# jumerckx/Monodepth2.jl

Measured on AMD Instinct MI355X. Metric: train-step images/sec, ResNet-18 416×128; 1/2/4/8 MI355X + roofline %, higher is better.
Workload: dtype fp32; 1 GPU; train_step resnet18 depth+pose decoders, 4-scale photometric loss, ADAM; batch_per_gpu=12, global_batch=12, height=128, width=416, parallelism=dp1

## Files before the change

include/md2.h:

```cpp
#ifndef MD2_H
#define MD2_H

#include <stddef.h>

#ifdef __cplusplus
extern "C" {
#endif

#define MD2_ABI_VERSION 2

#define MD2_OK 0
#define MD2_EINVAL 1
#define MD2_EHIP 2
#define MD2_ENOTSUP 3
#define MD2_ENOMEM 4
#define MD2_ESTATE 5

int md2_abi_version(void);
const char* md2_build_id(void);
const char* md2_last_error(void);
int md2_device_count(int* count);
int md2_memcpy_d2d(void* dst, const void* src, size_t bytes, void* stream);

#define MD2_MAX_SCALES 5
// ... 54 lines not shown
                        void* stream);
int md2_project_fwd(const float* points, int n, int w, int h, const float* K, const float* R,
                    const float* t, float* out, void* stream);
size_t md2_project_workspace_size(int n, int w, int h);
int md2_project_bwd(const float* points, int n, int w, int h, const float* K, const float* R,
                    const float* t, const float* dout, float* d_points, float* d_R, float* d_t,
                    void* workspace, void* stream);
int md2_grid_sample_border_fwd(const float* x, const float* grid, int n, int c, int hi, int wi,
                               int ho, int wo, float* out, void* stream);
int md2_grid_sample_border_bwd(const float* x, const float* grid, const float* dout, int n, int c,
                               int hi, int wi, int ho, int wo, float* d_grid, float* d_x,
                               void* stream);
size_t md2_smooth_loss_workspace_size(int n, int w, int h);
int md2_smooth_loss_fwd(const float* disp, const float* img, int n, int c, int h, int w,
                        float* loss, void* workspace, void* stream);
int md2_smooth_loss_bwd(const float* disp, const float* img, int n, int c, int h, int w,
                        float dloss, float* d_disp, void* workspace, void* stream);

typedef struct md2_warp_cfg {
  int n, c, width, height;
  int dw, dh;
  float K[9], invK[9];
  float min_depth, max_depth;
  long long x_sample_stride;
  long long x_frame_stride;
  int target, src0, src1;
} md2_warp_cfg;
size_t md2_warp_photometric_workspace_size(const md2_warp_cfg* cfg);
int md2_warp_photometric_fwd(const md2_warp_cfg* cfg, const float* disp, const float* Rt,
                             const float* x, const float* automask, float* loss_map,
                             signed char* sel_map, void* workspace, void* stream);
int md2_warp_photometric_bwd(const md2_warp_cfg* cfg, const float* disp, const float* Rt,
                             const float* x, const float* automask, const float* d_loss,
                             float* d_disp, float* d_Rt, void* workspace, void* stream);

int md2_png_info(const char* path, int* width, int* height, int* channels);
int md2_load_triplets_u8(const char* const* paths, int n, int width, int height,
                         const unsigned char* flip, unsigned char* out, int threads);
int md2_load_kitti_u8(const char* const* paths, int n, int height, int width,
                      const unsigned char* flip, unsigned char* out, int threads);

int md2_unorm8_to_float(const unsigned char* in, float* out, long long n, void* stream);

typedef struct md2_conv_desc {
  int n, cin, h, w, cout, kh, kw, stride, pad, reflect;
  int act;
} md2_conv_desc;

size_t md2_conv2d_workspace_size(const md2_conv_desc* d);
int md2_conv2d_fwd(const md2_conv_desc* d, const float* x, const float* w, const float* bias,
                   float* y, void* workspace, void* stream);
int md2_conv2d_dgrad(const md2_conv_desc* d, const float* dy, const float* w, float* dx,
                     void* workspace, void* stream);
int md2_conv2d_wgrad(const md2_conv_desc* d, const float* x, const float* dy, float* dw,
                     float* db, void* workspace, void* stream);
int md2_act_backward(const float* out, const float* dout, float* dpre, long long n, int act,
                     void* stream);

int md2_maxpool3s2_fwd(const float* x, int n, int c, int h, int w, float* y, unsigned char* arg,
                       void* stream);
int md2_maxpool3s2_bwd(const float* dy, const unsigned char* arg, int n, int c, int h, int w,
                       float* dx, void* stream);
int md2_upsample2_fwd(const float* x, int n, int c, int h, int w, float* y, void* stream);
int md2_upsample2_bwd(const float* dy, int n, int c, int h, int w, float* dx, void* stream);

int md2_mpi_embed_features(const float* feat, long long sample_stride, int n, int c, int h, int w,
                           const float* bins, int num_bins, int L, float* out, void* stream);
int md2_concat_channels(const float* a, int ca, const float* b, int cb, int n, long long hw,
                        float* out, void* stream);

int md2_mine_src_xyz(const float* disparity, int n_planes, int batch, int h, int w,
                     const float* invK, float* xyz, void* stream);
int md2_mine_tgt_xyz(const float* xyz_src, const float* pose, int n_planes, int batch, int h, int w,
                     float* xyz_tgt, void* stream);
int md2_mine_sample(const float* src, int c, const float* depth, const float* pose, int n_planes,
                    int batch, int h, int w, const float* K, const float* invK, float* out,
                    float* valid, void* stream);
int md2_plane_volume_rendering(const float* rgb, const float* sigma, const float* xyz, int n_planes,
                               int batch, int h, int w, float* rgb_out, float* transparency_acc,
                               float* weights, void* stream);
int md2_render_tgt_rgb_depth(const float* rgb, const float* sigma, const float* disparity,
                             const float* xyz_tgt, const float* pose, const float* invK,
                             const float* K, int n_planes, int batch, int h, int w, float* rgb_out,
                             float* depth, float* mask, void* stream);

typedef struct md2_model_cfg {
  int arch;
  int in_channels;
  int batch;
  int width, height;
  int n_levels;
  int scale_levels[MD2_MAX_SCALES];
  float K[9], invK[9];
  float min_depth, max_depth, disparity_smoothness;
  float scales[MD2_MAX_SCALES];
  int automasking;
  int target, src0, src1;
  int embedding_levels;
  int num_bins;
} md2_model_cfg;

typedef struct md2_model md2_model;

int md2_arch_param_count(const md2_model_cfg* cfg, long long* n_entries, long long* n_elems);
int md2_arch_param_info(const md2_model_cfg* cfg, int idx, char* name, int name_len, int* ndim,
                        int* shape4, long long* offset);
// ... 85 lines not shown
```

monodepth2.jl_amd/csrc/api.cpp:

```cpp
#include "../../include/md2.h"

#include <cmath>
#include <cstdlib>
#include <cstring>
#include <string>

#include "conv.h"
#include "loss_tail.h"
#include "mine.h"
#include "model.h"
#include "nn.h"

#include <algorithm>

#include <dlfcn.h>
#include <execinfo.h>
#include <csignal>
#include <unistd.h>

namespace md2 {
static struct sigaction g_prev_segv, g_prev_abrt;
static void segv_trace(int sig, siginfo_t* info, void* uctx) {
  void* frames[64];
  const int n = backtrace(frames, 64);
// ... 170 lines not shown
                        float* d_pose, void* stream) {
  MD2_CHECK_ARG(pose && dRt && d_pose && n > 0, "so3 bwd args");
  return launch_so3_bwd(pose, 2 * n, n, invert_mask, dRt, d_pose, 0, (hipStream_t)stream);
}

static ConvShape to_shape(const md2_conv_desc* d) {
  ConvShape s{};
  s.N = d->n;
  s.Cin = d->cin;
  s.H = d->h;
  s.W = d->w;
  s.Cout = d->cout;
  s.KH = d->kh;
  s.KW = d->kw;
  s.stride = d->stride;
  s.pad = d->pad;
  s.reflect = d->reflect;
  s.Ho = (d->h + 2 * d->pad - d->kh) / d->stride + 1;
  s.Wo = (d->w + 2 * d->pad - d->kw) / d->stride + 1;
  return s;
}

static size_t align_up(size_t b) { return (b + 255) & ~size_t(255); }

size_t md2_conv2d_workspace_size(const md2_conv_desc* d) {
  if (!d) return 0;
  const ConvShape s = to_shape(d);
  size_t packed = std::max(conv_fwd_packed_elems(s), conv_dgrad_packed_elems(s)) * sizeof(float);
  size_t slab = std::max(conv_fwd_workspace(s), std::max(conv_dgrad_workspace(s), conv_wgrad_workspace(s)));
  return align_up(packed) + align_up(slab);
}

int md2_conv2d_fwd(const md2_conv_desc* d, const float* x, const float* w, const float* bias,
                   float* y, void* workspace, void* stream) {
  MD2_CHECK_ARG(d && x && w && y && workspace, "conv2d_fwd args");
  const ConvShape s = to_shape(d);
  hipStream_t st = (hipStream_t)stream;
  float* packed = (float*)workspace;
  const size_t pbytes = align_up(std::max(conv_fwd_packed_elems(s), conv_dgrad_packed_elems(s)) * sizeof(float));
  MD2_TRY(conv_pack_fwd(s, w, packed, st));
  TensorIn in;
  in.p0 = x;
  in.c0 = s.Cin;
  in.bs0 = (long)s.Cin * s.H * s.W;
  TensorOut out;
  out.p0 = y;
  out.bs0 = (long)s.Cout * s.Ho * s.Wo;
  out.bias = bias;
  out.act = d->act;
  ConvWorkspace ws{(char*)workspace + pbytes, md2_conv2d_workspace_size(d) - pbytes};
  return conv_fwd(s, in, packed, out, ws, st);
}

int md2_conv2d_dgrad(const md2_conv_desc* d, const float* dy, const float* w, float* dx,
                     void* workspace, void* stream) {
  MD2_CHECK_ARG(d && dy && w && dx && workspace, "conv2d_dgrad args");
  const ConvShape s = to_shape(d);
  hipStream_t st = (hipStream_t)stream;
  float* packed = (float*)workspace;
  const size_t pbytes = align_up(std::max(conv_fwd_packed_elems(s), conv_dgrad_packed_elems(s)) * sizeof(float));
  MD2_TRY(conv_pack_dgrad(s, w, packed, st));
  TensorOut out;
  out.p0 = dx;
  out.bs0 = (long)s.Cin * s.H * s.W;
  ConvWorkspace ws{(char*)workspace + pbytes, md2_conv2d_workspace_size(d) - pbytes};
  return conv_dgrad(s, dy, packed, out, ws, st);
}

int md2_conv2d_wgrad(const md2_conv_desc* d, const float* x, const float* dy, float* dw,
                     float* db, void* workspace, void* stream) {
  MD2_CHECK_ARG(d && x && dy && dw && workspace, "conv2d_wgrad args");
  const ConvShape s = to_shape(d);
  const size_t pbytes = align_up(std::max(conv_fwd_packed_elems(s), conv_dgrad_packed_elems(s)) * sizeof(float));
  TensorIn in;
  in.p0 = x;
  in.c0 = s.Cin;
  in.bs0 = (long)s.Cin * s.H * s.W;
  ConvWorkspace ws{(char*)workspace + pbytes, md2_conv2d_workspace_size(d) - pbytes};
  return conv_wgrad(s, in, dy, dw, db, 0, ws, (hipStream_t)stream);
}

int md2_act_backward(const float* out, const float* dout, float* dpre, long long n, int act,
                     void* stream) {
  MD2_CHECK_ARG(out && dout && dpre && n >= 0, "act_backward args");
  return act_backward(out, dout, dpre, (long)n, act, (hipStream_t)stream);
}

int md2_adam(float* p, const float* g, float* adam_m, float* adam_v, long long n, float lr,
             float beta1, float beta2, float eps, int step, float grad_scale, void* stream) {
  MD2_CHECK_ARG(p && g && adam_m && adam_v && n > 0 && step >= 1, "adam args");
  const double bc1 = 1.0 - std::pow((double)beta1, step), bc2 = 1.0 - std::pow((double)beta2, step);
  return adam_step(p, g, adam_m, adam_v, (long)n, lr, beta1, beta2, eps, (float)bc1, (float)bc2,
                   grad_scale, (hipStream_t)stream);
}

int md2_maxpool3s2_fwd(const float* x, int n, int c, int h, int w, float* y, unsigned char* arg,
                       void* stream) {
  MD2_CHECK_ARG(x && y && arg && n > 0 && c > 0 && h > 0 && w > 0, "maxpool3s2_fwd args");
  return maxpool_fwd(x, n, c, h, w, y, arg, (h + 1) / 2, (w + 1) / 2, (hipStream_t)stream);
}
int md2_maxpool3s2_bwd(const float* dy, const unsigned char* arg, int n, int c, int h, int w,
                       float* dx, void* stream) {
  MD2_CHECK_ARG(dy && arg && dx && n > 0 && c > 0 && h > 0 && w > 0, "maxpool3s2_bwd args");
  return maxpool_bwd(dy, arg, n, c, h, w, (h + 1) / 2, (w + 1) / 2, dx, (hipStream_t)stream);
}
int md2_upsample2_fwd(const float* x, int n, int c, int h, int w, float* y, void* stream) {
  MD2_CHECK_ARG(x && y && n > 0 && c > 0 && h > 0 && w > 0, "upsample2_fwd args");
  return upsample2_fwd(x, n, c, h, w, y, (hipStream_t)stream);
}
int md2_mpi_embed_features(const float* feat, long long sample_stride, int n, int c, int h, int w,
                           const float* bins, int num_bins, int L, float* out, void* stream) {
  MD2_CHECK_ARG(feat && bins && out && n > 0 && c > 0 && h > 0 && w > 0 && num_bins > 0 && L >= 0 &&
                    sample_stride >= (long long)c * h * w, "mpi_embed_features args");
  return mpi_embed_features(feat, (long)sample_stride, n, c, h, w, bins, num_bins, L, out,
                            (hipStream_t)stream);
}
int md2_concat_channels(const float* a, int ca, const float* b, int cb, int n, long long hw,
                        float* out, void* stream) {
  MD2_CHECK_ARG(a && b && out && ca > 0 && cb > 0 && n > 0 && hw > 0, "concat_channels args");
// ... 306 lines not shown
```

monodepth2.jl_amd/csrc/conv.hip:

```cpp
#include "conv_plan.h"
#include "conv_lds.h"

namespace md2 {

struct PackOne {
  const float* w;
  float* out;
  int mode, tap, layout, Cout, Cin, KK, Kpad, Mpad;
  int Cinw;
};

__device__ __forceinline__ long packed_index(int k, int m, int layout, int Mpad) {
  return layout ? ((long)(k >> 4) * Mpad + m) * 16 + (k & 15) : (long)k * Mpad + m;
}
__device__ __forceinline__ void pack_store(float* out, int k, int m, int layout, int Mpad, float v) {
  if (layout == 2) {
    uint16_t* o = reinterpret_cast<uint16_t*>(out);
    uint32_t h, md, l;
    split3(v, h, md, l);
    const long base = ((long)(k >> 4) * 3 * Mpad + m) * 16 + (k & 15), ps = (long)Mpad * 16;
    o[base] = (uint16_t)(h >> 16);
    o[base + ps] = (uint16_t)(md >> 16);
    o[base + 2 * ps] = (uint16_t)(l >> 16);
  } else {
// ... 200 lines not shown
  return p;
}

HaloPlan plan_halo(const ConvShape& s, int mode) {
  HaloPlan h;
  static const int on = tuning_knob("MD2_HALO", 1);
  static const int target = tuning_knob("MD2_HX_TARGET", 256);
  if (!on || mode > 1 || s.KH != 3 || s.KW != 3 || s.stride != 1 || s.pad != 1 || (s.reflect && mode == 1)) return h;
  if (!conv_px3_used(s, mode) || !conv_tap_major(s, mode)) return h;
  const int M = mode == 0 ? s.Cout : s.Cin, C = mode == 0 ? s.Cin : s.Cout;
  if (C % 16 || s.cin_w) return h;
  const int hrmax = Halo3Lds::rows(s.W);
  const bool flat = M % 64 == 0 && Halo3Lds::fits(s.W) && cdiv((long)hrmax * s.W, 512) <= 2;
  static const int d2on = tuning_knob("MD2_HALO2D", 1);
  const bool d2 = !flat && (d2on >> mode & 1) && M % 32 == 0 && tuning_knob("MD2_PX3_TERMS", 6) != 9 &&
                  2L * s.H * s.W >= (long)round_up(s.H, 8) * round_up(s.W, 32);
  if (!flat && !d2) return h;
  long tiles;
  int tgt = target;
  if (flat) {
    h.items = cdiv((long)hrmax * s.W, 512);
    tiles = (long)(M / 64) * cdiv((long)s.N * s.H * s.W, 256);
  } else {
    h.d2 = true;
    h.mw = M % 64 == 0 ? 2 : 1;
    tiles = (long)(M / (32 * h.mw)) * s.N * cdiv(s.H, 8) * cdiv(s.W, 32);
    tgt = h.mw == 1 ? 2 * target : target;
  }
  const int nch = C / 16;
  int splits = 1;
  while (tiles * splits * 2 <= tgt && nch / (splits * 2) >= 2) splits *= 2;
  h.cper = cdiv(nch, splits);
  h.splits = cdiv(nch, h.cper);
  h.ok = true;
  return h;
}

HaloS2Plan plan_halo_s2(const ConvShape& s) {
  HaloS2Plan h;
  static const int on = tuning_knob("MD2_HALO_S2", 1);
  if (!on || s.KH != 3 || s.KW != 3 || s.stride != 2 || s.pad != 1 || s.reflect || s.cin_w) return h;
  if (s.H != 2 * s.Ho || s.W != 2 * s.Wo || s.Cin % 64 || s.Cout % 16) return h;
  if (!conv_px3_used(s, 1) || !conv_tap_major(s, 1) || tuning_knob("MD2_PX3_TERMS", 6) == 9) return h;
  if (!Halo3s2Lds::fits(s.Wo)) return h;
  h.items = 1;
  const long tiles = (long)(s.Cin / 64) * cdiv((long)s.N * s.Ho * s.Wo, 128);
  const int nch = s.Cout / 16;
  int splits = 1;
  while (tiles * splits * 2 <= 256 && nch / (splits * 2) >= 2) splits *= 2;
  h.cper = cdiv(nch, splits);
  h.splits = cdiv(nch, h.cper);
  h.ok = true;
  return h;
}

WHaloPlan plan_whalo(const ConvShape& s, int c0) {
  WHaloPlan h;
  static const int on = tuning_knob("MD2_WHALO", 1);
  static const int target = tuning_knob("MD2_WHX_TARGET", 256);
  if (!on || s.KH != 3 || s.KW != 3 || s.stride != 1 || s.pad != 1 || s.reflect) return h;
  if (s.Cin % 32 || s.Cout % 64 || c0 < s.Cin || (s.cin_w && s.cin_w != s.Cin) || s.W > 112) return h;
  if (tuning_knob("MD2_PX3_TERMS", 6) == 9) return h;
  int r = 0;
  for (int d = 1; d <= s.H; ++d)
    if (s.H % d == 0 && d * s.W <= 112) r = d;
  if (r == 0 || (r * s.W) % 4 || (s.H * s.W) % 4 || r * s.W < 49) return h;
  if (!WHaloLds::fits(r, s.W)) return h;
  static const int maxit = tuning_knob("MD2_WHX_MAXITEMS", 4);
  h.items = cdiv(4L * (r + 2) * s.W, 384);
  if (h.items > std::min(4, maxit)) return h;
  h.r = r;
  h.nchunk = s.N * s.H / r;
  const long tiles = (long)(s.Cin / 32) * (s.Cout / 64);
  long splits = std::max(1L, (long)target / tiles);
  splits = std::min(splits, std::max(1L, (long)h.nchunk / 2));
  h.cper = cdiv(h.nchunk, splits);
  h.splits = cdiv(h.nchunk, h.cper);
  h.ok = true;
  return h;
}

ConvShape reflect_ext_shape(const ConvShape& s) {
  ConvShape e = s;
  e.H = s.H + 2;
  e.W = s.W + 2;
  e.Ho = e.H;
  e.Wo = e.W;
  e.reflect = 0;
  return e;
}
bool reflect_dgrad_on_halo(const ConvShape& s, HaloPlan* hp) {
  static const int on = tuning_knob("MD2_HALO_RFL_DGRAD", 1);
  if (!on || !s.reflect || s.KH != 3 || s.stride != 1 || s.pad != 1 || s.cin_w || s.H < 2 || s.W < 2) return false;
  const HaloPlan h = plan_halo(reflect_ext_shape(s), 1);
  if (hp) *hp = h;
  return h.ok;
}
size_t reflect_dgrad_ws(const ConvShape& s) {
  HaloPlan h;
  if (!reflect_dgrad_on_halo(s, &h)) return 0;
  const long Ne = (long)s.N * (s.H + 2) * (s.W + 2);
  return ((size_t)(h.splits > 1 ? h.splits : 0) + 1) * s.Cin * Ne * sizeof(float);
}

int wgrad_cw(const ConvShape& s, int c0, int BN) {
  for (int cw = 128; cw >= 16; cw /= 2)
// ... 328 lines not shown
```

monodepth2.jl_amd/csrc/conv_dgrad.hip:

```cpp
#include "conv_px_launch.h"

namespace md2 {

template <bool SMALL>
__global__ __launch_bounds__(256) void fold_reflect_kernel(const float* __restrict__ src, int splits, long ss,
                                                           long sn, long sc, TensorOut o, FastDiv fd_hw,
                                                           FastDiv fd_w, FastDiv fd_c, uint32_t total) {
  constexpr int NR = SMALL ? 3 : 2;
  const uint32_t idx = blockIdx.x * 256u + threadIdx.x;
  if (idx >= total) return;
  const int H = (int)fd_hw.d / (int)fd_w.d, W = (int)fd_w.d, P = W + 2;
  const uint32_t nc = fdiv(idx, fd_hw);
  const int pix = (int)(idx - nc * fd_hw.d);
  const int n = (int)fdiv(nc, fd_c), c = (int)(nc - n * fd_c.d);
  const int i = (int)fdiv((uint32_t)pix, fd_w), j = pix - i * W;
  const float* p = src + n * sn + c * sc;
  const int rows[3] = {i + 1, i == 1 ? 0 : (i == H - 2 ? H + 1 : -1), (i == H - 2 && i == 1) ? H + 1 : -1};
  const int cols[3] = {j + 1, j == 1 ? 0 : (j == W - 2 ? W + 1 : -1), (j == W - 2 && j == 1) ? W + 1 : -1};
  int off[NR * NR];
  bool use[NR * NR];
#pragma unroll
  for (int a_ = 0; a_ < NR; ++a_)
#pragma unroll
    for (int b_ = 0; b_ < NR; ++b_) {
// ... 127 lines not shown
    const bool sl = df.slab != nullptr;
    const long total = (long)s.N * s.Cin * s.H * s.W;
    const bool small = s.H == 3 || s.W == 3;
    static const int f4on = tuning_knob("MD2_FOLD4", 1);
    const bool f4 = f4on && !small && s.W % 4 == 0 && s.H >= 4 && s.W >= 8 && ((long)s.H * s.W) % 4 == 0 &&
                    ((uintptr_t)dx.p0 % 16) == 0 && dx.bs0 % 4 == 0 &&
                    (!dx.p1 || (((uintptr_t)dx.p1 % 16) == 0 && dx.bs1 % 4 == 0));
    if (f4)
      hipLaunchKernelGGL(fold_reflect4_kernel<0>, dim3(cdiv(total / 4, 256)), dim3(256), 0, st,
                         sl ? df.slab : dxp, sl ? df.splits : 1, (long)s.Cin * Ne, sl ? HWp : s.Cin * HWp,
                         sl ? Ne : HWp, dx, make_fastdiv((uint32_t)(s.H * s.W)),
                         make_fastdiv((uint32_t)(s.W / 4)), make_fastdiv((uint32_t)s.Cin), s.H,
                         (uint32_t)(total / 4));
    else
      hipLaunchKernelGGL(small ? fold_reflect_kernel<true> : fold_reflect_kernel<false>, dim3(cdiv(total, 256)),
                         dim3(256), 0, st, sl ? df.slab : dxp, sl ? df.splits : 1, (long)s.Cin * Ne,
                         sl ? HWp : s.Cin * HWp, sl ? Ne : HWp, dx, make_fastdiv((uint32_t)(s.H * s.W)),
                         make_fastdiv((uint32_t)s.W), make_fastdiv((uint32_t)s.Cin), (uint32_t)total);
    MD2_LAUNCH_CHECK();
    return MD2_OK;
  }
  if (const HaloS2Plan h2 = plan_halo_s2(s); h2.ok) {
    ConvArgs ak = a;
    ak.g.N = (long)s.N * s.Ho * s.Wo;
    ak.fd_pix = make_fastdiv((uint32_t)(s.Ho * s.Wo));
    ak.fd_row = make_fastdiv((uint32_t)s.Wo);
    ak.hx_cper = h2.cper;
    ak.slab = nullptr;
    if (h2.splits > 1) {
      const size_t need = (size_t)h2.splits * a.g.M * a.g.N * sizeof(float);
      MD2_CHECK_ARG(ws.ptr && ws.bytes >= need, "conv_dgrad: stride-2 halo workspace too small");
      ak.slab = (float*)ws.ptr;
    }
    conv_arith_ref() = 6;
    MD2_TRY(halo_s2_launch(ak, h2.items, h2.splits, st));
    if (h2.splits > 1) {
      ConvArgs ar = a;
      ar.slab = ak.slab;
      const TensorOut& o = a.out;
      const bool aligned4 = a.fd_pix.d % 4 == 0 && o.bs0 % 4 == 0 && (!o.p1 || o.bs1 % 4 == 0) &&
                            ((uintptr_t)o.p0 % 16) == 0 && (!o.p1 || ((uintptr_t)o.p1 % 16) == 0);
      const long total = (long)a.g.M * a.g.N;
      MD2_CHECK_ARG(total < (1L << 31), "conv_dgrad: split-K reduction index exceeds 2^31");
      if (aligned4)
        hipLaunchKernelGGL(splitk_reduce_px4_kernel<0>, dim3(cdiv(total / 4, 256)), dim3(256), 0, st, ar,
                           h2.splits);
      else
        hipLaunchKernelGGL(splitk_reduce_px_kernel<0>, dim3(cdiv(total, 256)), dim3(256), 0, st, ar,
                           h2.splits, 0, make_fastdiv((uint32_t)a.g.N), make_fastdiv((uint32_t)total));
      MD2_LAUNCH_CHECK();
    }
    return MD2_OK;
  }
  if (s.stride == 2 && conv_tap_major(s, 1) && conv_px2_used(s, 1) && s.KH <= 3 && s.H % 2 == 0 &&
      s.W % 2 == 0) {
    ConvArgs ac = a;
    int kmax = 0;
    for (int cls = 0; cls < 4; ++cls) {
      const PhaseClass c = phase_class(s, cls >> 1, cls & 1);
      ac.ph_y0c[cls] = c.y0;
      ac.ph_x0c[cls] = c.x0;
      ac.ph_ntc[cls] = c.ntaps;
      for (int t = 0; t < 4; ++t) ac.ph_taps[4 * cls + t] = t < c.ntaps ? c.taps[t] : 0;
      kmax = std::max(kmax, c.ntaps);
      if (cls == 0) {
        ac.g.N = (long)s.N * c.Hc * c.Wc;
        ac.fd_pix = make_fastdiv((uint32_t)(c.Hc * c.Wc));
        ac.fd_row = make_fastdiv((uint32_t)c.Wc);
      }
    }
    ac.g.K = kmax * s.Cout;
    ac.ph_S = 1;
    const Plan p = plan_px(ac.g.M, 4 * ac.g.N, ac.g.K, s.Cout % 32 == 0, true);
    return launch_px<1>(s, ac, p, ws, st);
  }
  if (s.stride == 2 && conv_tap_major(s, 1)) {
    for (int cls = 0; cls < 4; ++cls) {
      const PhaseClass c = phase_class(s, cls >> 1, cls & 1);
      if (c.Hc <= 0 || c.Wc <= 0 || (c.ntaps == 0 && dx.accumulate)) continue;
      ConvArgs ac = a;
      ac.ph_y0 = c.y0;
      ac.ph_x0 = c.x0;
      for (int t = 0; t < 16; ++t) ac.ph_taps[t] = t < c.ntaps ? c.taps[t] : 0;
      ac.g.N = (long)s.N * c.Hc * c.Wc;
      ac.g.K = c.ntaps * s.Cout;
      ac.fd_pix = make_fastdiv((uint32_t)(c.Hc * c.Wc));
      ac.fd_row = make_fastdiv((uint32_t)c.Wc);
      const Plan p = plan_px(ac.g.M, ac.g.N, ac.g.K, s.Cout % 32 == 0);
      MD2_TRY(launch_px<1>(s, ac, p, ws, st));
    }
    return MD2_OK;
  }
  const Plan p = plan_px(a.g.M, a.g.N, a.g.K, conv_tap_major(s, 1) && s.Cout % 32 == 0);
  return launch_px<1>(s, a, p, ws, st, defer);
}

}
```

monodepth2.jl_amd/csrc/conv_fwd.hip:

```cpp
#include "conv_px_launch.h"

namespace md2 {

int conv_fwd(const ConvShape& s, const TensorIn& x, const float* wpacked, const TensorOut& y,
             ConvWorkspace ws, hipStream_t st, SplitKDefer* defer) {
  if (defer) {
    const SplitKDefer req = *defer;
    *defer = SplitKDefer{};
    defer->stats = req.stats;
    defer->keep_reduce = req.keep_reduce;
  }
  MD2_TRY(check_shape(s));
  MD2_CHECK_ARG(x.p0 && wpacked && y.p0, "conv_fwd pointers");
  MD2_CHECK_ARG(x.c0 == s.Cin || x.p1 != nullptr, "conv_fwd: second input tensor missing");
  MD2_CHECK_ARG(x.c0 >= s.Cin || !conv_tap_major(s, 0) || x.c0 % 16 == 0,
                "conv_fwd: concat split must be a multiple of 16 channels");
  if (head_path(s) && x.c0 >= s.Cin && y.c0 >= 1) {
    MD2_CHECK_ARG(!conv_px2_used(s, 0), "head: packed layout");
    conv_arith_ref() = 0;
    return head_fwd(s, conv_head_in(x), conv_head_w(s, 0, wpacked), y.bias, y.act, y.p0, y.bs0,
                    y.accumulate, st);
  }
  ConvArgs a{};
  fill_common(a, s);
  a.g.M = s.Cout;
  a.g.N = (long)s.N * s.Ho * s.Wo;
  a.g.K = s.Cin * s.KH * s.KW;
  a.g.Mpad = (int)round_up(s.Cout, MPAD);
  a.fd_pix = make_fastdiv((uint32_t)(s.Ho * s.Wo));
  a.fd_row = make_fastdiv((uint32_t)s.Wo);
  a.fd_bdiv = make_fastdiv((uint32_t)std::min(x.bdiv, 1 << 30));
  a.in = x;
  a.A = wpacked;
  a.out = y;
  a.A_bytes = (uint32_t)(conv_fwd_packed_elems(s) * sizeof(float));
  {
    long ext0 = 0;
    for (int b = 0; b < s.N; ++b)
      ext0 = std::max(ext0, (long)(b % x.bdiv) * x.bs0 + (long)(b / x.bdiv) * x.bhi);
    ext0 += (long)x.c0 * s.H * s.W;
    const long ext1 = x.p1 ? (long)(s.N - 1) * x.bs1 + (long)(s.Cin - x.c0) * s.H * s.W : 0;
    MD2_CHECK_ARG(ext0 * 4 < (long)OOB && ext1 * 4 < (long)OOB, "conv_fwd: tensor exceeds 2 GB");
    a.b0_bytes = (uint32_t)(ext0 * 4);
    a.b1_bytes = (uint32_t)(ext1 * 4);
  }
  if (stem_s2d_applies(s, x, y)) {
    conv_arith_ref() = 6;
    return stem_s2d_launch(s, a, st);
  }
  const bool bk32 = conv_tap_major(s, 0) && s.Cin % 32 == 0 && (x.c0 >= s.Cin || x.c0 % 32 == 0);
  const Plan p = plan_px(a.g.M, a.g.N, a.g.K, bk32);
  return launch_px<0>(s, a, p, ws, st, defer);
}

}
```

monodepth2.jl_amd/csrc/conv_lds.h:

```cpp
#pragma once

#ifdef __HIPCC__
#define MD2_LDS_FN __host__ __device__ __forceinline__ constexpr
#else
#define MD2_LDS_FN constexpr
#endif

namespace md2 {

constexpr int HX_PAD = 16;

template <int PX, int TN>
struct HaloFlatLds {
  static constexpr int plane = PX * 32;
  static constexpr long cap = 6L * plane;
  MD2_LDS_FN static long bytes() { return cap; }
  MD2_LDS_FN static int pitch(int W) { return W + HX_PAD; }
  MD2_LDS_FN static int rows(int W) { return (TN - 1) / W + 4; }
  MD2_LDS_FN static int zero_px(int HR, int W) { return HR * pitch(W); }
  MD2_LDS_FN static long pixels(int W) { return (long)rows(W) * pitch(W) + 3; }
  MD2_LDS_FN static long need(int W) { return 5L * plane + pixels(W) * 32; }
  MD2_LDS_FN static bool fits(int W) { return pixels(W) <= PX; }
};
constexpr int HX_PX = 736;
constexpr int HS2_PX = 416;
using Halo3Lds = HaloFlatLds<HX_PX, 256>;
using Halo3s2Lds = HaloFlatLds<HS2_PX, 128>;
constexpr int HX_PLANE = Halo3Lds::plane;
constexpr int HS2_PLANE = Halo3s2Lds::plane;

constexpr int H2_TH = 8, H2_TW = 32, H2_HR = H2_TH + 2, H2_PR = H2_TW + 2;
constexpr int H2_PX = H2_HR * H2_PR;
constexpr int H2_PLANE = H2_PX * 32;
struct Halo2dLds {
  static constexpr long cap = 6L * H2_PLANE;
  MD2_LDS_FN static long bytes() { return cap; }
  MD2_LDS_FN static long need() { return cap; }
  MD2_LDS_FN static bool fits() { return true; }
};

struct WHaloLds {
  static constexpr long cap = 65536;
  static constexpr int KS_MAX = 7;
  MD2_LDS_FN static int pitch(int W) { return W + 2; }
  MD2_LDS_FN static int zero_px(int r, int W) { return (r + 2) * pitch(W); }
  MD2_LDS_FN static int plane(int zero_px) { return (zero_px + 3) * 64; }
  MD2_LDS_FN static int ktab(int plane) { return 3 * plane; }
  MD2_LDS_FN static long need(int r, int W, int ksteps) { return (long)ktab(plane(zero_px(r, W))) + 16L * ksteps * 4; }
  MD2_LDS_FN static long bytes(int r, int W) { return need(r, W, KS_MAX); }
  MD2_LDS_FN static bool fits(int r, int W) { return bytes(r, W) <= cap; }
};

struct StemRingLds {
  static constexpr long cap = 163840;
  MD2_LDS_FN static int plane(int P) { return 5 * P * 32; }
  MD2_LDS_FN static long ring(int P) { return 3L * 5 * P * 32; }
};
struct StemLds : StemRingLds {
  MD2_LDS_FN static int pitch(int Wo) { return Wo + 3; }
  MD2_LDS_FN static long bytes(int P) { return ring(P); }
  MD2_LDS_FN static long need(int P) { return ring(P); }
  MD2_LDS_FN static bool fits(int Wo) { return bytes(pitch(Wo)) <= cap; }
};
struct StemWgradLds : StemRingLds {
  static constexpr int TILES = 13;
  static constexpr int red_quarter = TILES * 4 * 64;
  static constexpr long red_bytes = 4L * red_quarter * 4;
  MD2_LDS_FN static int pitch(int Wo) { return ((Wo + 31) / 32 * 32 + 3 + 7) / 8 * 8; }
  MD2_LDS_FN static long need(int P) { return ring(P) > red_bytes ? ring(P) : red_bytes; }
  MD2_LDS_FN static long bytes(int P) { return need(P); }
  MD2_LDS_FN static bool fits(int Wo) { return pitch(Wo) <= 512 && ring(pitch(Wo)) <= cap; }
};

}
```

monodepth2.jl_amd/csrc/conv_plan.h:

```cpp
#pragma once
#include "conv_kernel.h"
#include "head.h"

namespace md2 {

constexpr int TARGET_BLOCKS = 1536;

enum TileCfg { T128x128 = 0, T64x256 = 1, T32x256 = 2, T64x128 = 3, T128x64 = 4, T64x64 = 5, T32x128 = 6,
               T128x64q = 7 };
const int TILE_BM[] = {128, 64, 32, 64, 128, 64, 32, 128};
const int TILE_BN[] = {128, 256, 256, 128, 64, 64, 128, 64};

enum WTileCfg { W64x128 = 0, W32x256 = 1, W64x64 = 2, W32x128 = 3, W16x144 = 4, WSTEM = 5, W64x192 = 6 };
const int WT_BM[] = {64, 32, 64, 32, 16, 64, 64};
const int WT_BN[] = {128, 256, 64, 128, 144, 64, 192};

#define MD2_CONV_COMBOS(X) X(1, 1, 0) X(1, 2, 0) X(3, 1, 0) X(3, 1, 1) X(3, 2, 0) X(7, 2, 0)

struct Plan {
  int tile;
  int BM, BN, BK;
  int splits;
  int kper;
};
struct HaloPlan {
  bool ok = false;
  int items = 0, splits = 1, cper = 1;
  bool d2 = false;
  int mw = 2;
};
struct HaloS2Plan {
  bool ok = false;
  int items = 0, splits = 1, cper = 1;
};
struct WHaloPlan {
  bool ok = false;
  int r = 0, items = 0, nchunk = 0, splits = 1, cper = 1;
};
struct WPlan {
  int tile, BM, BN;
  int cw;
  long ntiles_n;
  int splits, kper;
};
struct PhaseClass {
  int y0, x0, Hc, Wc, ntaps;
  int taps[16];
};

Plan plan_px(int M, long N, int K, bool bk32_ok = false, bool prefer32 = false);
HaloPlan plan_halo(const ConvShape& s, int mode);
HaloS2Plan plan_halo_s2(const ConvShape& s);
WHaloPlan plan_whalo(const ConvShape& s, int c0);
WPlan plan_wgrad(const ConvShape& s, int c0);
int wgrad_cw(const ConvShape& s, int c0, int BN);
ConvShape reflect_ext_shape(const ConvShape& s);
bool reflect_dgrad_on_halo(const ConvShape& s, HaloPlan* hp = nullptr);
size_t reflect_dgrad_ws(const ConvShape& s);
PhaseClass phase_class(const ConvShape& s, int cy, int cx);
void fill_common(ConvArgs& a, const ConvShape& s);
int check_shape(const ConvShape& s);
int px3_terms();
int bias_parts(int C, long total);
bool head_path(const ConvShape& s);

int halo_launch(int mode, const ConvArgs& a, int items, int splits, int reflect, hipStream_t st);
int halo2d_launch(int mode, const ConvArgs& a, int mw, int splits, int reflect, hipStream_t st);
int halo_s2_launch(const ConvArgs& a, int items, int splits, hipStream_t st);
int whalo_launch(const ConvArgs& a, int items, int ksteps, int splits, hipStream_t st);
bool stem_s2d_applies(const ConvShape& s, const TensorIn& x, const TensorOut& y);
int stem_s2d_launch(const ConvShape& s, const ConvArgs& a, hipStream_t st);
bool stem_wgrad_s2d_applies(const ConvShape& s, const TensorIn& x);
int stem_wgrad_blocks(const ConvShape& s);
int stem_wgrad_s2d_launch(const ConvShape& s, const ConvArgs& a, hipStream_t st);

}
```

monodepth2.jl_amd/md2hip/ops.py:

```python
from __future__ import annotations

import ctypes as C

from . import _lib
from ._lib import ConvDesc, check, lib, ptr, stream_of

ACT = {None: 0, "identity": 0, "relu": 1, "elu": 2, "sigmoid": 3}


def conv_desc(x_shape, w_shape, stride=1, pad=0, reflect=False, act=None) -> ConvDesc:
    n, cin, h, w = x_shape
    cout, cin2, kh, kw = w_shape
    if cin != cin2:
        raise ValueError(f"channel mismatch {cin} vs {cin2}")
    d = ConvDesc()
    d.n, d.cin, d.h, d.w, d.cout, d.kh, d.kw = n, cin, h, w, cout, kh, kw
    d.stride, d.pad, d.reflect, d.act = stride, pad, int(reflect), ACT[act]
    return d


def _ws(d, dev):
    import torch
    nbytes = lib().md2_conv2d_workspace_size(C.byref(d))
    return torch.empty(max(nbytes // 4, 1) + 64, dtype=torch.float32, device=dev)


def out_hw(h, w, k, stride, pad):
    return (h + 2 * pad - k) // stride + 1, (w + 2 * pad - k) // stride + 1


def conv2d(x, weight, bias=None, stride=1, pad=0, reflect=False, act=None):
    import torch
    d = conv_desc(tuple(x.shape), tuple(weight.shape), stride, pad, reflect, act)
    ho, wo = out_hw(d.h, d.w, d.kh, stride, pad)
    y = torch.empty(d.n, d.cout, ho, wo, dtype=torch.float32, device=x.device)
    check(lib().md2_conv2d_fwd(C.byref(d), ptr(x), ptr(weight), ptr(bias), ptr(y),
                               ptr(_ws(d, x.device)), stream_of(x.device)), "md2_conv2d_fwd")
    return y


def conv2d_dgrad(dy, weight, x_shape, stride=1, pad=0, reflect=False):
    import torch
    d = conv_desc(tuple(x_shape), tuple(weight.shape), stride, pad, reflect)
    dx = torch.empty(*x_shape, dtype=torch.float32, device=dy.device)
    check(lib().md2_conv2d_dgrad(C.byref(d), ptr(dy), ptr(weight), ptr(dx), ptr(_ws(d, dy.device)),
                                 stream_of(dy.device)), "md2_conv2d_dgrad")
    return dx


def conv2d_wgrad(x, dy, w_shape, stride=1, pad=0, reflect=False, bias=True):
    import torch
    d = conv_desc(tuple(x.shape), tuple(w_shape), stride, pad, reflect)
    dw = torch.empty(*w_shape, dtype=torch.float32, device=x.device)
    db = torch.empty(w_shape[0], dtype=torch.float32, device=x.device) if bias else None
    check(lib().md2_conv2d_wgrad(C.byref(d), ptr(x), ptr(dy), ptr(dw), ptr(db), ptr(_ws(d, x.device)),
                                 stream_of(x.device)), "md2_conv2d_wgrad")
    return dw, db


def act_backward(out, dout, act):
    import torch
    dpre = torch.empty_like(dout)
    check(lib().md2_act_backward(ptr(out), ptr(dout), ptr(dpre), dout.numel(), ACT[act],
                                 stream_of(out.device)), "md2_act_backward")
    return dpre


def maxpool3s2(x):
    import torch
    n, c, h, w = x.shape
    y = torch.empty(n, c, (h + 1) // 2, (w + 1) // 2, dtype=torch.float32, device=x.device)
    arg = torch.empty(y.shape, dtype=torch.uint8, device=x.device)
    check(lib().md2_maxpool3s2_fwd(ptr(x), n, c, h, w, ptr(y), ptr(arg), stream_of(x.device)),
          "md2_maxpool3s2_fwd")
    return y, arg


def maxpool3s2_backward(dy, arg, x_shape):
    import torch
    n, c, h, w = x_shape
    dx = torch.empty(n, c, h, w, dtype=torch.float32, device=dy.device)
    check(lib().md2_maxpool3s2_bwd(ptr(dy), ptr(arg), n, c, h, w, ptr(dx), stream_of(dy.device)),
          "md2_maxpool3s2_bwd")
    return dx


def upsample2(x):
    import torch
    n, c, h, w = x.shape
    y = torch.empty(n, c, 2 * h, 2 * w, dtype=torch.float32, device=x.device)
    check(lib().md2_upsample2_fwd(ptr(x), n, c, h, w, ptr(y), stream_of(x.device)),
          "md2_upsample2_fwd")
    return y


def upsample2_backward(dy):
    import torch
    n, c, h2, w2 = dy.shape
    dx = torch.empty(n, c, h2 // 2, w2 // 2, dtype=torch.float32, device=dy.device)
# ... 4 lines not shown
```

Baseline: 1922 images/s.

## Add dedicated 1x1 conv GEMM kernel with bf16x3 MFMA for fwd and dgrad

Adds a specialized kernel for 1x1 convolutions (ResNet downsample shortcuts) that treats them as a plain GEMM. Inputs are split into three bf16 parts and computed with six MFMA products, double-buffered through LDS. It is used for forward when the tile count and channel count are small, and for dgrad. Stride-2 dgrad writes zeros into the skipped pixels in place of a separate clear. It also adds an accumulate dgrad entry point. The aim is to replace the general implicit-GEMM path, which has poor occupancy on these small layers, at the cost of more code paths and plan heuristics.

```diff
diff --git a/include/md2.h b/include/md2.h
--- a/include/md2.h
+++ b/include/md2.h
@@ -130,6 +130,8 @@
                    float* y, void* workspace, void* stream);
 int md2_conv2d_dgrad(const md2_conv_desc* d, const float* dy, const float* w, float* dx,
                      void* workspace, void* stream);
+int md2_conv2d_dgrad_accumulate(const md2_conv_desc* d, const float* dy, const float* w, float* dx,
+                                void* workspace, void* stream);
 int md2_conv2d_wgrad(const md2_conv_desc* d, const float* x, const float* dy, float* dw,
                      float* db, void* workspace, void* stream);
 int md2_act_backward(const float* out, const float* dout, float* dpre, long long n, int act,
diff --git a/monodepth2.jl_amd/csrc/api.cpp b/monodepth2.jl_amd/csrc/api.cpp
--- a/monodepth2.jl_amd/csrc/api.cpp
+++ b/monodepth2.jl_amd/csrc/api.cpp
@@ -246,8 +246,8 @@
   return conv_fwd(s, in, packed, out, ws, st);
 }
 
-int md2_conv2d_dgrad(const md2_conv_desc* d, const float* dy, const float* w, float* dx,
-                     void* workspace, void* stream) {
+static int conv2d_dgrad_impl(const md2_conv_desc* d, const float* dy, const float* w, float* dx,
+                             int accumulate, void* workspace, void* stream) {
   MD2_CHECK_ARG(d && dy && w && dx && workspace, "conv2d_dgrad args");
   const ConvShape s = to_shape(d);
   hipStream_t st = (hipStream_t)stream;
@@ -257,8 +257,19 @@
   TensorOut out;
   out.p0 = dx;
   out.bs0 = (long)s.Cin * s.H * s.W;
+  out.accumulate = accumulate;
   ConvWorkspace ws{(char*)workspace + pbytes, md2_conv2d_workspace_size(d) - pbytes};
   return conv_dgrad(s, dy, packed, out, ws, st);
+}
+
+int md2_conv2d_dgrad(const md2_conv_desc* d, const float* dy, const float* w, float* dx,
+                     void* workspace, void* stream) {
+  return conv2d_dgrad_impl(d, dy, w, dx, 0, workspace, stream);
+}
+
+int md2_conv2d_dgrad_accumulate(const md2_conv_desc* d, const float* dy, const float* w, float* dx,
+                                void* workspace, void* stream) {
+  return conv2d_dgrad_impl(d, dy, w, dx, 1, workspace, stream);
 }
 
 int md2_conv2d_wgrad(const md2_conv_desc* d, const float* x, const float* dy, float* dw,
diff --git a/monodepth2.jl_amd/csrc/conv.hip b/monodepth2.jl_amd/csrc/conv.hip
--- a/monodepth2.jl_amd/csrc/conv.hip
+++ b/monodepth2.jl_amd/csrc/conv.hip
@@ -276,6 +276,29 @@
   h.splits = cdiv(nch, h.cper);
   h.ok = true;
   return h;
+}
+
+Gemm1Plan plan_gemm1(const ConvShape& s, int mode) {
+  Gemm1Plan g;
+  static const int on = tuning_knob("MD2_GEMM1", 1);
+  if (!on || mode > 1 || s.KH != 1 || s.KW != 1 || s.pad != 0 || s.reflect || s.cin_w) return g;
+  if (!conv_px3_used(s, mode) || !conv_tap_major(s, mode) || px3_terms() != 6) return g;
+  const int M = mode == 0 ? s.Cout : s.Cin, C = mode == 0 ? s.Cin : s.Cout;
+  if (M % 64 || C % 16) return g;
+  constexpr long G1_TARGET = 192;
+  const long P = (long)s.N * s.Ho * s.Wo;
+  constexpr long G1_FWD_TILES = 384, G1_FWD_K = 256;
+  if (mode == 0 && ((long)(M / 64) * cdiv(P, 64) >= G1_FWD_TILES || C > G1_FWD_K)) return g;
+  auto fits = [&](int tn) {
+    return tn == 128 ? Gemm1Lds<128>::fits(C) : tn == 64 ? Gemm1Lds<64>::fits(C) : Gemm1Lds<32>::fits(C);
+  };
+  for (int tn = 128; tn >= 32; tn /= 2) {
+    if (!fits(tn)) continue;
+    g.tn = tn;
+    if ((long)(M / 64) * cdiv(P, tn) >= G1_TARGET) break;
+  }
+  g.ok = g.tn > 0;
+  return g;
 }
 
 WHaloPlan plan_whalo(const ConvShape& s, int c0) {
diff --git a/monodepth2.jl_amd/csrc/conv_dgrad.hip b/monodepth2.jl_amd/csrc/conv_dgrad.hip
--- a/monodepth2.jl_amd/csrc/conv_dgrad.hip
+++ b/monodepth2.jl_amd/csrc/conv_dgrad.hip
@@ -203,6 +203,14 @@
     }
     return MD2_OK;
   }
+  if (const Gemm1Plan g1 = plan_gemm1(s, 1); g1.ok) {
+    ConvArgs ak = a;
+    ak.g.N = (long)s.N * s.Ho * s.Wo;
+    ak.fd_pix = make_fastdiv((uint32_t)(s.Ho * s.Wo));
+    ak.fd_row = make_fastdiv((uint32_t)s.Wo);
+    conv_arith_ref() = 6;
+    return gemm1_launch(1, ak, g1.tn, st);
+  }
   if (s.stride == 2 && conv_tap_major(s, 1) && conv_px2_used(s, 1) && s.KH <= 3 && s.H % 2 == 0 &&
       s.W % 2 == 0) {
     ConvArgs ac = a;
diff --git a/monodepth2.jl_amd/csrc/conv_fwd.hip b/monodepth2.jl_amd/csrc/conv_fwd.hip
--- a/monodepth2.jl_amd/csrc/conv_fwd.hip
+++ b/monodepth2.jl_amd/csrc/conv_fwd.hip
@@ -48,6 +48,11 @@
     conv_arith_ref() = 6;
     return stem_s2d_launch(s, a, st);
   }
+  if (const Gemm1Plan g1 = plan_gemm1(s, 0); g1.ok && x.c0 >= s.Cin && x.bdiv >= s.N) {
+    if (defer) *defer = SplitKDefer{};
+    conv_arith_ref() = 6;
+    return gemm1_launch(0, a, g1.tn, st);
+  }
   const bool bk32 = conv_tap_major(s, 0) && s.Cin % 32 == 0 && (x.c0 >= s.Cin || x.c0 % 32 == 0);
   const Plan p = plan_px(a.g.M, a.g.N, a.g.K, bk32);
   return launch_px<0>(s, a, p, ws, st, defer);
diff --git a/monodepth2.jl_amd/csrc/conv_gemm1.hip b/monodepth2.jl_amd/csrc/conv_gemm1.hip
--- /dev/null
+++ b/monodepth2.jl_amd/csrc/conv_gemm1.hip
@@ -0,0 +1,5 @@
+#include "conv_plan.h"
+#include "conv_lds.h"
+namespace md2 {
+#include "conv_gemm1.inc"
+}
diff --git a/monodepth2.jl_amd/csrc/conv_gemm1.inc b/monodepth2.jl_amd/csrc/conv_gemm1.inc
--- /dev/null
+++ b/monodepth2.jl_amd/csrc/conv_gemm1.inc
@@ -0,0 +1,178 @@
+
+__device__ __forceinline__ uint32_t g1_swz(uint32_t off) { return off ^ ((off >> 4) & 16u); }
+
+__device__ __forceinline__ float* g1_out_ptr(const TensorOut& o, int m, int img, long pix, long plane) {
+  return (m < o.c0) ? o.p0 + (long)img * o.bs0 + (long)m * plane + pix
+                    : o.p1 + (long)img * o.bs1 + (long)(m - o.c0) * plane + pix;
+}
+
+template <int MODE, int WN>
+__global__ __launch_bounds__(128 * WN, 2) void conv_gemm1_kernel(ConvArgs a) {
+  static_assert(WN == 1 || WN == 2 || WN == 4, "waves along N");
+  constexpr int NT = 128 * WN, TN = 32 * WN;
+  static_assert(NT / TN == G1_CHUNKS, "a group is staged by one pass of the block: one chunk per thread");
+  using L = Gemm1Lds<TN>;
+  extern __shared__ __attribute__((aligned(16))) uint8_t lds[];
+
+  const int tid = threadIdx.x, lane = tid & 63;
+  const int wq = __builtin_amdgcn_readfirstlane(tid >> 6);
+  const int wm = wq / WN, wn = wq % WN;
+  const int fi = lane & 31, fh = lane >> 5;
+  const int S = a.stride;
+  const uint32_t N = (uint32_t)a.g.N;
+  const uint32_t n0 = blockIdx.x * (uint32_t)TN;
+  const int m0 = blockIdx.y * 64;
+  const int nch = (MODE == 0 ? a.Cin : a.Cout) >> 4;
+  const int ngr = (nch + G1_CHUNKS - 1) / G1_CHUNKS;
+
+  const int sp = tid % TN, sq = tid / TN;
+  const uint32_t ch4 = MODE == 0 ? a.HW4 : a.HoWo4;
+  uint32_t goff = OOB;
+  {
+    const uint32_t n = n0 + (uint32_t)sp;
+    if (n < N) {
+      const uint32_t img = fdiv(n, a.fd_pix);
+      const uint32_t r = n - img * a.fd_pix.d;
+      if (MODE == 0) {
+        const uint32_t y = fdiv(r, a.fd_row), x = r - y * a.fd_row.d;
+        goff = (img * (uint32_t)a.in.bs0 + (uint32_t)S * (y * (uint32_t)a.W + x)) * 4u;
+      } else {
+        goff = (img * (uint32_t)(a.Cout * a.HoWo) + r) * 4u;
+      }
+    }
+  }
+  const uint32_t loff = g1_swz((uint32_t)sp * 32u);
+
+  const __amdgpu_buffer_rsrc_t rA = make_rsrc(a.A, a.A_bytes);
+  const __amdgpu_buffer_rsrc_t rB = make_rsrc(MODE == 0 ? (const void*)a.in.p0 : (const void*)a.dy, a.b0_bytes);
+  const uint32_t apart = (uint32_t)a.g.Mpad * 32u;
+  const uint32_t achunk = 3u * apart;
+  const uint32_t aoff = (uint32_t)(((m0 + wm * 32 + fi) * 16 + 8 * fh) * 2);
+
+  float stg[16];
+  u32x4_t af[G1_CHUNKS][3];
+  f32x16 acc0, acc1;
+#pragma unroll
+  for (int r = 0; r < 16; ++r) acc0[r] = acc1[r] = 0.f;
+
+  auto stage_load = [&](int g) {
+    const uint32_t c = (uint32_t)(g * G1_CHUNKS + sq);
+    const uint32_t voff = goff == OOB ? OOB : goff + c * 16u * ch4;
+#pragma unroll
+    for (int ch = 0; ch < 16; ++ch) stg[ch] = bload_s(rB, voff, (uint32_t)ch * ch4);
+  };
+  auto stage_write = [&](int buf) {
+    uint32_t hm[3][8];
+#pragma unroll
+    for (int p = 0; p < 8; ++p) split3_pk(stg[2 * p], stg[2 * p + 1], hm[0][p], hm[1][p], hm[2][p]);
+#pragma unroll
+    for (int q = 0; q < 3; ++q) {
+      uint8_t* dst = lds + (buf * 3 + q) * L::plane + sq * L::chunk;
+      *reinterpret_cast<u32x4_t*>(dst + loff) = u32x4_t{hm[q][0], hm[q][1], hm[q][2], hm[q][3]};
+      *reinterpret_cast<u32x4_t*>(dst + (loff ^ 16u)) = u32x4_t{hm[q][4], hm[q][5], hm[q][6], hm[q][7]};
+    }
+  };
+  auto load_a = [&](int g) {
+#pragma unroll
+    for (int cl = 0; cl < G1_CHUNKS; ++cl) {
+      const uint32_t base = (uint32_t)(g * G1_CHUNKS + cl) * achunk + aoff;
+#pragma unroll
+      for (int q = 0; q < 3; ++q) af[cl][q] = bload16(rA, base + (uint32_t)q * apart);
+    }
+  };
+
+  stage_load(0);
+  load_a(0);
+  stage_write(0);
+  __syncthreads();
+
+  const uint32_t boff = g1_swz((uint32_t)(wn * 32 + fi) * 32u + 16u * (uint32_t)fh);
+
+  for (int g = 0; g < ngr; ++g) {
+    const int cur = g & 1;
+    const bool more = g + 1 < ngr;
+    const uint8_t* img = lds + cur * 3 * L::plane;
+    const int ncg = min(G1_CHUNKS, nch - g * G1_CHUNKS);
+    if (more) stage_load(g + 1);
+    __builtin_amdgcn_sched_barrier(0);
+#pragma unroll
+    for (int cl = 0; cl < G1_CHUNKS; ++cl) {
+      if (cl >= ncg) break;
+      const bf16x8_t ah = __builtin_bit_cast(bf16x8_t, af[cl][0]);
+      const bf16x8_t am = __builtin_bit_cast(bf16x8_t, af[cl][1]);
+      const bf16x8_t al = __builtin_bit_cast(bf16x8_t, af[cl][2]);
+      const uint8_t* src = img + cl * L::chunk + boff;
+      const bf16x8_t bh = __builtin_bit_cast(bf16x8_t, *reinterpret_cast<const u32x4_t*>(src));
+      const bf16x8_t bm = __builtin_bit_cast(bf16x8_t, *reinterpret_cast<const u32x4_t*>(src + L::plane));
+      const bf16x8_t bl = __builtin_bit_cast(bf16x8_t, *reinterpret_cast<const u32x4_t*>(src + 2 * L::plane));
+      f32x16 c = acc1;
+      c = __builtin_amdgcn_mfma_f32_32x32x16_bf16(am, bm, c, 0, 0, 0);
+      c = __builtin_amdgcn_mfma_f32_32x32x16_bf16(al, bh, c, 0, 0, 0);
+      c = __builtin_amdgcn_mfma_f32_32x32x16_bf16(ah, bl, c, 0, 0, 0);
+      c = __builtin_amdgcn_mfma_f32_32x32x16_bf16(am, bh, c, 0, 0, 0);
+      c = __builtin_amdgcn_mfma_f32_32x32x16_bf16(ah, bm, c, 0, 0, 0);
+      acc1 = c;
+      acc0 = __builtin_amdgcn_mfma_f32_32x32x16_bf16(ah, bh, acc0, 0, 0, 0);
+    }
+    __builtin_amdgcn_sched_barrier(0);
+    if (more) {
+      load_a(g + 1);
+      stage_write(cur ^ 1);
+    }
+    __syncthreads();
+  }
+
+  const uint32_t nn = n0 + (uint32_t)(wn * 32 + fi);
+  if (nn >= N) return;
+  if (MODE == 0 || S == 1) {
+    int img;
+    long pix, plane;
+    out_pixel(a, false, (long)nn, img, pix, plane);
+#pragma unroll
+    for (int r = 0; r < 16; ++r) {
+      const int m = m0 + wm * 32 + (r & 3) + 8 * (r >> 2) + 4 * fh;
+      store_out(a.out, m, img, pix, plane, acc0[r] + acc1[r]);
+    }
+  } else {
+    const uint32_t img = fdiv(nn, a.fd_pix);
+    const uint32_t rr = nn - img * a.fd_pix.d;
+    const uint32_t y = fdiv(rr, a.fd_row), x = rr - y * a.fd_row.d;
+    const long pix = (long)(2 * y) * a.W + 2 * x;
+    const bool right = 2 * (int)x + 1 < a.W, below = 2 * (int)y + 1 < a.H;
+    const bool zero = !a.out.accumulate;
+#pragma unroll
+    for (int r = 0; r < 16; ++r) {
+      const int m = m0 + wm * 32 + (r & 3) + 8 * (r >> 2) + 4 * fh;
+      store_out(a.out, m, (int)img, pix, a.HW, acc0[r] + acc1[r]);
+      if (zero) {
+        float* d = g1_out_ptr(a.out, m, (int)img, pix, a.HW);
+        if (right) d[1] = 0.f;
+        if (below) d[a.W] = 0.f;
+        if (right && below) d[a.W + 1] = 0.f;
+      }
+    }
+  }
+}
+
+template <int MODE, int WN>
+static int gemm1_launch_as(const ConvArgs& a, hipStream_t st) {
+  constexpr int TN = 32 * WN;
+  using L = Gemm1Lds<TN>;
+  const int C = MODE == 0 ? a.Cin : a.Cout;
+  const dim3 grid(cdiv(a.g.N, TN), a.g.M / 64), block(128 * WN);
+  const LdsSize z{L::need(C), L::bytes(C), L::cap};
+  return lds_launch<conv_gemm1_kernel<MODE, WN>>(grid, block, z, st, a);
+}
+template <int MODE>
+static int gemm1_launch_mode(const ConvArgs& a, int tn, hipStream_t st) {
+  switch (tn) {
+    case 128: return gemm1_launch_as<MODE, 4>(a, st);
+    case 64: return gemm1_launch_as<MODE, 2>(a, st);
+    case 32: return gemm1_launch_as<MODE, 1>(a, st);
+  }
+  set_error("conv_gemm1: no kernel for this pixel tile");
+  return MD2_EINVAL;
+}
+int gemm1_launch(int mode, const ConvArgs& a, int tn, hipStream_t st) {
+  return mode == 0 ? gemm1_launch_mode<0>(a, tn, st) : gemm1_launch_mode<1>(a, tn, st);
+}
diff --git a/monodepth2.jl_amd/csrc/conv_lds.h b/monodepth2.jl_amd/csrc/conv_lds.h
--- a/monodepth2.jl_amd/csrc/conv_lds.h
+++ b/monodepth2.jl_amd/csrc/conv_lds.h
@@ -72,4 +72,18 @@
   MD2_LDS_FN static bool fits(int Wo) { return pitch(Wo) <= 512 && ring(pitch(Wo)) <= cap; }
 };
 
+constexpr int G1_CHUNKS = 4;
+template <int TN>
+struct Gemm1Lds {
+  static_assert(TN == 32 || TN == 64 || TN == 128, "conv_gemm1 pixel tiles");
+  static constexpr int chunk = TN * 32;
+  static constexpr int plane = G1_CHUNKS * chunk;
+  static constexpr long cap = 6L * plane;
+  MD2_LDS_FN static int groups(int C) { return (C / 16 + G1_CHUNKS - 1) / G1_CHUNKS; }
+  MD2_LDS_FN static int buffers(int C) { return groups(C) > 1 ? 2 : 1; }
+  MD2_LDS_FN static long bytes(int C) { return 3L * plane * buffers(C); }
+  MD2_LDS_FN static long need(int C) { return 3L * plane * buffers(C); }
+  MD2_LDS_FN static bool fits(int C) { return C > 0 && C % 16 == 0 && bytes(C) <= cap; }
+};
+
 }
diff --git a/monodepth2.jl_amd/csrc/conv_plan.h b/monodepth2.jl_amd/csrc/conv_plan.h
--- a/monodepth2.jl_amd/csrc/conv_plan.h
+++ b/monodepth2.jl_amd/csrc/conv_plan.h
@@ -33,6 +33,10 @@
   bool ok = false;
   int items = 0, splits = 1, cper = 1;
 };
+struct Gemm1Plan {
+  bool ok = false;
+  int tn = 0;
+};
 struct WHaloPlan {
   bool ok = false;
   int r = 0, items = 0, nchunk = 0, splits = 1, cper = 1;
@@ -51,6 +55,7 @@
 Plan plan_px(int M, long N, int K, bool bk32_ok = false, bool prefer32 = false);
 HaloPlan plan_halo(const ConvShape& s, int mode);
 HaloS2Plan plan_halo_s2(const ConvShape& s);
+Gemm1Plan plan_gemm1(const ConvShape& s, int mode);
 WHaloPlan plan_whalo(const ConvShape& s, int c0);
 WPlan plan_wgrad(const ConvShape& s, int c0);
 int wgrad_cw(const ConvShape& s, int c0, int BN);
@@ -68,6 +73,7 @@
 int halo2d_launch(int mode, const ConvArgs& a, int mw, int splits, int reflect, hipStream_t st);
 int halo_s2_launch(const ConvArgs& a, int items, int splits, hipStream_t st);
 int whalo_launch(const ConvArgs& a, int items, int ksteps, int splits, hipStream_t st);
+int gemm1_launch(int mode, const ConvArgs& a, int tn, hipStream_t st);
 bool stem_s2d_applies(const ConvShape& s, const TensorIn& x, const TensorOut& y);
 int stem_s2d_launch(const ConvShape& s, const ConvArgs& a, hipStream_t st);
 bool stem_wgrad_s2d_applies(const ConvShape& s, const TensorIn& x);
diff --git a/monodepth2.jl_amd/md2hip/ops.py b/monodepth2.jl_amd/md2hip/ops.py
--- a/monodepth2.jl_amd/md2hip/ops.py
+++ b/monodepth2.jl_amd/md2hip/ops.py
@@ -45,6 +45,15 @@
     dx = torch.empty(*x_shape, dtype=torch.float32, device=dy.device)
     check(lib().md2_conv2d_dgrad(C.byref(d), ptr(dy), ptr(weight), ptr(dx), ptr(_ws(d, dy.device)),
                                  stream_of(dy.device)), "md2_conv2d_dgrad")
+    return dx
+
+
+def conv2d_dgrad_accumulate(dy, weight, dx, stride=1, pad=0, reflect=False):
+    from ._lib import declare
+    declare("md2_conv2d_dgrad_accumulate", C.c_int, [C.POINTER(ConvDesc)] + [C.c_void_p] * 5)
+    d = conv_desc(tuple(dx.shape), tuple(weight.shape), stride, pad, reflect)
+    check(lib().md2_conv2d_dgrad_accumulate(C.byref(d), ptr(dy), ptr(weight), ptr(dx), ptr(_ws(d, dy.device)),
+                                            stream_of(dy.device)), "md2_conv2d_dgrad_accumulate")
     return dx
 
 
```

After: 1925 images/s, median of 6. No clear change (+0.2%).
